# Illumina/manta

Hardware: AMD Instinct MI355X
Metric: candidate SV loci assembled+aligned per second (whole node) (higher is better)
Workload: dtype int32; 1 GPU; BASELINE config[1]: synthetic small-indel loci, 80 reads/locus x150bp, k=31..76 step 5, assemble + 10-mer trim + GlobalLargeIndelAligner(2,-8,-24,-1,-1;-100) on 1800 bp windows; loci_per_gpu=10000, reads_per_locus=80, block_loci=10000, workers_per_gpu=1, parallelism=loci sharded over 1 rank(s); per rank a cost-ordered block queue, queue=rank, dist_world=1, mix=False

## Files before the change

manta_amd/csrc/align_pair.hpp:

```cpp
#pragma once
#include "align_kernels.hpp"

namespace manta_dev {

static const int PAIR_BAD8 = -32768;

WV_HD bool pairEligible(const int E, const int match, const int mismatch, const int open, const int extend, const int offEdge,
                        const int largeIndel, const int allowEdgeIns)
{
  if (E > 6 || allowEdgeIns) return false;
  const long q      = 64L * E;
  const long perCol = -long((mismatch < offEdge) ? ((mismatch < 0) ? mismatch : 0) : ((offEdge < 0) ? offEdge : 0));
  const long gaps   = -long((open < 0) ? open : 0) - long((extend < 0) ? extend : 0) - long((largeIndel < 0) ? largeIndel : 0);
  const long up     = q * long((match > 0) ? match : 0);
  if (open > 0 || extend > 0 || largeIndel > 0 || match < 0 || match > 64 || mismatch < -512 || offEdge < -512 || open < -2048 || largeIndel < -2048 || extend < -512)
    return false;
  const long liftJD = (largeIndel - open > 0) ? long(largeIndel - open) : 0L;
  return q * perCol + gaps + up + liftJD + 64 < 4096;
}

template <int E>
struct PairAligner {
  static const int   NS = 5;
  const AlignParams& P;

  WV_DEV PairAligner(const AlignParams& p) : P(p) {}

  WV_DEV static uint32_t pk(const int lo, const int hi) { return (uint32_t(lo) & 0xffffu) | (uint32_t(hi) << 16); }
  WV_DEV static uint32_t pk2(const int v) { return pk(v, v); }
  WV_DEV static int      half(const uint32_t v, const int h) { return h ? (int(v) >> 16) : int(int16_t(v & 0xffffu)); }

  WV_DEV void sweep(const AlignTaskDev& TA, const AlignTaskDev& TB, uint32_t* ptr32, StartCand& outA, StartCand& outB)
  {
    const int      lane = wv::lane();
    const unsigned QA = TA.query_len, QB = TB.query_len, GA = TA.ref1_len, GB = TB.ref1_len;
    const unsigned G  = (GA > GB) ? GA : GB;
    const int      open = P.open, extend = P.extend, L = P.extra, offEdge = P.off_edge;
    const uint32_t cM0 = pk2(7), cD1 = pk2(6), cI2 = pk2(5), cJ3 = pk2(4), cJI4 = pk2(3);
    const uint32_t cOpen0   = pk2(open * 8 + 7);
    const uint32_t cL0      = pk2(L * 8 + 7);
    const uint32_t cLmOpen2 = pk2((L - open) * 8 + 5);
    const uint32_t cL4      = pk2(L * 8 + 3);
    const uint32_t cBad1 = pk2(PAIR_BAD8 + 6), cBad3 = pk2(PAIR_BAD8 + 4);
    const uint32_t cExt     = pk2(extend * 8);
    const uint32_t cMatch   = pk2(P.match * 8);
    const uint32_t cMisDiff = pk2((P.mismatch - P.match) * 8);
    const uint32_t clrIdx = 0xfff8fff8u, idxBits = 0x00070007u, bad = pk2(PAIR_BAD8);

    const unsigned Qs[2] = {QA, QB}, Gs[2] = {GA, GB};
    unsigned       lQ[2], eQ[2];
    for (int h = 0; h < 2; ++h) {
      lQ[h] = (Qs[h] - 1) / E;
      eQ[h] = (Qs[h] - 1) % E;
    }
    int      rowKey[2] = {int(0x80000000u), int(0x80000000u)};
    uint32_t lastRow[E];
    for (int e = 0; e < E; ++e) lastRow[e] = bad;
    const uint32_t fcMask = (lane == 0) ? 0xffffffffu : 0u;

    uint32_t st[NS][E], lcur[NS], lprev[NS], qc[E];
    for (int e = 0; e < E; ++e) {
      const unsigned q0 = unsigned(lane) * E + e;
      const unsigned a = (q0 < QA) ? TA.query[q0] : 0u, b = (q0 < QB) ? TB.query[q0] : 0u;
      qc[e]            = a | (b << 16);
      const int row0   = int((q0 + 1) * unsigned(offEdge)) * 8;
      for (int s = 0; s < NS; ++s) st[s][e] = bad;
      st[ST_MATCH][e] = pk2(row0 < PAIR_BAD8 ? PAIR_BAD8 : row0);
    }
    for (int s = 0; s < NS; ++s) lcur[s] = lprev[s] = bad;
    lcur[ST_MATCH] = lprev[ST_MATCH] = 0;

    unsigned curA = 0, curB = 0, nextA = 0, nextB = 0;
    {
      const unsigned i0 = unsigned(lane);
      nextA             = (i0 < GA) ? TA.ref1[i0] : 0u;
      nextB             = (i0 < GB) ? TB.ref1[i0] : 0u;
    }
    uint32_t rc = 0;

    const unsigned nSteps = G + 63;
    for (unsigned t = 1; t <= nSteps; ++t) {
      if (((t - 1) & 63) == 0) {
        curA              = nextA;
        curB              = nextB;
        const unsigned i0 = t - 1 + 64 + unsigned(lane);
        nextA             = (i0 < GA) ? TA.ref1[i0] : 0u;
        nextB             = (i0 < GB) ? TB.ref1[i0] : 0u;
      }
      const unsigned c0 = wv::readlane(curA, int((t - 1) & 63)) | (wv::readlane(curB, int((t - 1) & 63)) << 16);
      rc                = wv::shr1(rc, c0);
      uint32_t incoming[NS];
      for (int s = 0; s < NS; ++s) incoming[s] = wv::shr1(st[s][E - 1], (s == ST_MATCH) ? 0u : bad);
      const int g = int(t) - lane;
      for (int s = 0; s < NS; ++s) {
        lprev[s] = lcur[s];
        lcur[s]  = incoming[s];
      }
      const bool active = (g >= 1) && (unsigned(g) <= G);
      if (!active) continue;

      uint32_t diag[NS], left[NS];
      for (int s = 0; s < NS; ++s) {
        diag[s] = lprev[s];
        left[s] = lcur[s];
      }
      uint32_t cells[E];
      for (int e = 0; e < E; ++e) {
        uint32_t up[NS];
        for (int s = 0; s < NS; ++s) up[s] = st[s][e];
        const uint32_t fc = (e == 0) ? fcMask : 0u;
        const uint32_t differ = wv::pk_min_u16(qc[e] ^ rc, 0x00010001u);
        const uint32_t sub8   = wv::pk_mad_u16(differ, cMisDiff, cMatch);
        uint32_t       nv[NS], code;
        {
          uint32_t m = wv::pk_max_i16(wv::pk_max_i16(wv::pk_add_sat_i16(diag[ST_MATCH], cM0), wv::pk_add_sat_i16(diag[ST_DELETE], cD1)), wv::pk_add_sat_i16(diag[ST_INSERT], cI2));
          m          = wv::pk_max_i16(wv::pk_max_i16(m, wv::pk_add_sat_i16(diag[ST_JUMP], cJ3)), wv::pk_add_sat_i16(diag[ST_JUMPINS], cJI4));
          nv[ST_MATCH] = wv::pk_add_sat_i16(m & clrIdx, sub8);
          code         = m & idxBits;
        }
        {
          uint32_t m = wv::pk_max_i16(wv::pk_max_i16(wv::pk_add_sat_i16(up[ST_MATCH], cOpen0), wv::pk_add_sat_i16(up[ST_DELETE], cD1)), wv::pk_add_sat_i16(up[ST_INSERT], cI2));
          m          = wv::pk_max_i16(wv::pk_max_i16(m, cBad3), wv::pk_add_sat_i16(up[ST_JUMPINS], cJI4));
          uint32_t b = wv::pk_add_sat_i16(m & clrIdx, cExt);
          b = (b & ~fc) | (bad & fc);
          nv[ST_DELETE] = b;
          code |= (m & idxBits) << 3;
        }
        {
          uint32_t m = wv::pk_max_i16(wv::pk_max_i16(wv::pk_add_sat_i16(left[ST_MATCH], cOpen0), cBad1), wv::pk_add_sat_i16(left[ST_INSERT], cI2));
          uint32_t b = wv::pk_add_sat_i16(m & clrIdx, cExt);
          b = (b & ~fc) | (bad & fc);
          nv[ST_INSERT] = b;
          code |= (m & idxBits) << 6;
        }
        {
          uint32_t m = wv::pk_max_i16(wv::pk_max_i16(wv::pk_add_sat_i16(up[ST_MATCH], cL0), cBad1), wv::pk_add_sat_i16(up[ST_INSERT], cLmOpen2));
          m          = wv::pk_max_i16(wv::pk_max_i16(m, wv::pk_add_sat_i16(up[ST_JUMP], cJ3)), wv::pk_add_sat_i16(up[ST_JUMPINS], cL4));
          uint32_t b = m & clrIdx;
          b = (b & ~fc) | (bad & fc);
          nv[ST_JUMP] = b;
          code |= (m & idxBits) << 9;
        }
        {
          uint32_t m = wv::pk_max_i16(wv::pk_max_i16(wv::pk_add_sat_i16(left[ST_MATCH], cL0), cBad1), wv::pk_add_sat_i16(left[ST_JUMPINS], cJI4));
          uint32_t b = m & clrIdx;
          b = (b & ~fc) | (bad & fc);
          nv[ST_JUMPINS] = b;
          code |= (m & idxBits) << 12;
        }
        for (int s = 0; s < NS; ++s) {
          diag[s]  = up[s];
          left[s]  = nv[s];
          st[s][e] = nv[s];
        }
        cells[e] = code;
      }
#ifndef MANTA_PAIR_EXPERIMENT_NO_STORE
      for (int e = 0; e < E; ++e) ptr32[(uint64_t(t) * E + e) * 64 + unsigned(lane)] = cells[e];
#else
      if (t == 0xffffffffu) for (int e = 0; e < E; ++e) ptr32[e] = cells[e];
#endif

      {
        const uint32_t cap = ((unsigned(g) == GA) ? 0x0000ffffu : 0u) | ((unsigned(g) == GB) ? 0xffff0000u : 0u);
        for (int e = 0; e < E; ++e) lastRow[e] = (lastRow[e] & ~cap) | (st[ST_MATCH][e] & cap);
        for (int h = 0; h < 2; ++h) {
          uint32_t vM = st[ST_MATCH][0];
          for (int e = 1; e < E; ++e) vM = (unsigned(e) == eQ[h]) ? st[ST_MATCH][e] : vM;
          const int  key = int((uint32_t(half(vM, h)) << 16) | (0xffffu - unsigned(g)));
          const bool on  = unsigned(lane) == lQ[h] && unsigned(g) <= Gs[h];
          rowKey[h]      = imax(rowKey[h], on ? key : int(0x80000000u));
        }
      }
    }
    for (int h = 0; h < 2; ++h) {
      bool     haveOff = false;
      int      offVal  = 0;
      unsigned offQ    = 0;
      for (int e = 0; e < E; ++e) {
        const unsigned q = unsigned(lane) * E + e + 1;
        if (q < Qs[h]) {
          const int v = (half(lastRow[e], h) >> 3) + int((Qs[h] - q) * unsigned(offEdge));
          if (!haveOff || v > offVal) {
            haveOff = true;
            offVal  = v;
            offQ    = q;
          }
        }
      }
      if (lane == 0) {
        const int v0 = int(Qs[h] * unsigned(offEdge));
        if (!haveOff || v0 >= offVal) {
          haveOff = true;
          offVal  = v0;
          offQ    = 0;
        }
      }
      waveArgmaxFirst(haveOff, offVal, offQ);
      const int key = wv::readlane(rowKey[h], int(lQ[h]));
      StartCand best;
      best.val   = (key >> 16) >> 3;
      best.ref   = 0xffffu - (unsigned(key) & 0xffffu);
      best.query = Qs[h];
      best.state = ST_MATCH;
      best.init  = true;
      candUpdate(best, offVal, Gs[h], offQ, ST_MATCH);
      if (h == 0)
        outA = best;
      else
        outB = best;
    }
  }

  WV_DEV void run(const AlignTaskDev& TA, const AlignTaskDev& TB, AlignResultDev& resA, AlignResultDev& resB, const bool haveB, uint8_t* slab)
  {
    StartCand sa, sb;
    sweep(TA, TB, reinterpret_cast<uint32_t*>(slab), sa, sb);
    wv::sync();
    for (int h = 0; h < (haveB ? 2 : 1); ++h) {
      const AlignTaskDev& T = h ? TB : TA;
      Aligner<1, E, true> al(P);
      al.query      = T.query;
      al.ref1       = T.ref1;
      al.ref2       = nullptr;
      al.Q          = T.query_len;
      al.R1         = T.ref1_len;
      al.R2         = 0;
      al.G          = T.ref1_len;
      al.ptr        = reinterpret_cast<uint16_t*>(slab) + h;
      al.nStrips    = 1;
      al.stripCells = 0;
      AlignResultDev r;
      al.tracebackSingle(h ? sb : sa, T, r);
      if (wv::lane() == 0) (h ? resB : resA) = r;
      wv::sync();
    }
  }
};

template <int E>
WV_KERNEL void align_pair_kernel(const AlignParams P)
{
  uint8_t*       slab   = P.ptr_ws + uint64_t(wv::block()) * P.ptr_ws_stride;
  const unsigned nTasks = P.n_tasks_dev ? *P.n_tasks_dev : P.n_tasks;
  const unsigned nPairs = (nTasks + 1) / 2;
  while (true) {
    unsigned slot = 0;
    if (wv::lane() == 0) slot = wv::atomic_add(P.counter, 1u);
    slot = wv::first(slot);
    if (slot >= nPairs) break;
    const unsigned ia = 2 * slot, ib = (2 * slot + 1 < nTasks) ? 2 * slot + 1 : 2 * slot;
    const unsigned ta = P.task_ids ? P.task_ids[ia] : ia, tb = P.task_ids ? P.task_ids[ib] : ib;
    PairAligner<E> al(P);
    al.run(P.tasks[ta], P.tasks[tb], P.results[ta], P.results[tb], ib != ia, slab);
    wv::sync();
  }
}

struct PairMultiParams {
  AlignParams     A;
  const uint32_t* bucket_ids;
  const uint32_t* counts;
  uint32_t        n_slots;
  uint32_t        n_order;
  uint8_t         order[8];
  uint8_t         e_of[8];
  uint32_t        prio_work[3];
};

template <int E>
WV_DEV void runPairWidth(const AlignParams& A, const unsigned ta, const unsigned tb, const bool haveB, uint8_t* slab)
{
  PairAligner<E>(A).run(A.tasks[ta], A.tasks[tb], A.results[ta], A.results[tb], haveB, slab);
}

#if !MANTA_TU_DEFINES(MANTA_TU_ALIGN_PAIR)
WV_KERNEL_OCC(4) void align_pair_multi_kernel(const PairMultiParams M);
#else
WV_KERNEL_OCC(4) void align_pair_multi_kernel(const PairMultiParams M)
{
  uint8_t* slab = M.A.ptr_ws + uint64_t(wv::block()) * M.A.ptr_ws_stride;
  unsigned n0 = 0, n1 = 0, n2 = 0, n3 = 0, n4 = 0, n5 = 0;
  if (M.n_order > 0) n0 = M.counts[M.order[0]];
  if (M.n_order > 1) n1 = M.counts[M.order[1]];
  if (M.n_order > 2) n2 = M.counts[M.order[2]];
  if (M.n_order > 3) n3 = M.counts[M.order[3]];
  if (M.n_order > 4) n4 = M.counts[M.order[4]];
  if (M.n_order > 5) n5 = M.counts[M.order[5]];
  const unsigned f1 = (n0 + 1) / 2, f2 = f1 + (n1 + 1) / 2, f3 = f2 + (n2 + 1) / 2, f4 = f3 + (n3 + 1) / 2, f5 = f4 + (n4 + 1) / 2,
                 f6 = f5 + (n5 + 1) / 2;
  while (true) {
    unsigned slot = 0;
    if (wv::lane() == 0) slot = wv::atomic_add(M.A.counter, 1u);
    slot = wv::first(slot);
    if (slot >= f6) break;
    unsigned j = 0, base = 0, n = n0;
    if (slot >= f1) { j = 1; base = f1; n = n1; }
    if (slot >= f2) { j = 2; base = f2; n = n2; }
    if (slot >= f3) { j = 3; base = f3; n = n3; }
    if (slot >= f4) { j = 4; base = f4; n = n4; }
    if (slot >= f5) { j = 5; base = f5; n = n5; }
    const unsigned  p   = slot - base;
    const uint32_t* ids = M.bucket_ids + uint64_t(M.order[j]) * M.n_slots;
    const unsigned  ia = 2 * p, ib = (2 * p + 1 < n) ? 2 * p + 1 : 2 * p;
    const unsigned  ta = ids[ia], tb = ids[ib];
    {
      const unsigned ga = M.A.tasks[ta].ref1_len, gb = M.A.tasks[tb].ref1_len;
      const unsigned work = unsigned(M.e_of[j]) * (((ga > gb) ? ga : gb) + 64u);
      wv::setprio((M.prio_work[2] && work >= M.prio_work[2]) ? 3u : (M.prio_work[1] && work >= M.prio_work[1]) ? 2u : (M.prio_work[0] && work >= M.prio_work[0]) ? 1u : 0u);
    }
    switch (M.e_of[j]) {
    case 1: runPairWidth<1>(M.A, ta, tb, ib != ia, slab); break;
    case 2: runPairWidth<2>(M.A, ta, tb, ib != ia, slab); break;
    case 3: runPairWidth<3>(M.A, ta, tb, ib != ia, slab); break;
    case 4: runPairWidth<4>(M.A, ta, tb, ib != ia, slab); break;
    case 5: runPairWidth<5>(M.A, ta, tb, ib != ia, slab); break;
    default: runPairWidth<6>(M.A, ta, tb, ib != ia, slab); break;
    }
    wv::sync();
  }
}
#endif

#if MANTA_TU != MANTA_TU_ALL
#if MANTA_TU == MANTA_TU_ALIGN_PAIR
#define MANTA_X
#else
#define MANTA_X extern
#endif
MANTA_X template __global__ void align_pair_kernel<1>(const AlignParams);
MANTA_X template __global__ void align_pair_kernel<2>(const AlignParams);
MANTA_X template __global__ void align_pair_kernel<3>(const AlignParams);
MANTA_X template __global__ void align_pair_kernel<4>(const AlignParams);
MANTA_X template __global__ void align_pair_kernel<5>(const AlignParams);
MANTA_X template __global__ void align_pair_kernel<6>(const AlignParams);
#undef MANTA_X
#endif

}
```

manta_amd/csrc/api.cpp:

```cpp
#include "api_internal.hpp"

extern "C" {

uint32_t manta_abi_version(void) { return MANTA_ABI_VERSION; }
uint64_t manta_batch_stats_size(void) { return sizeof(manta_batch_stats_t); }

int manta_ctx_create(int device_id, manta_ctx_t** out)
{
  if (!out) {
    g_createError = "manta_ctx_create: null output pointer";
    return MANTA_E_INVALID_ARG;
  }
  *out = nullptr;
  try {
    rt::init(device_id);
    if (!stringHashMatchesLibstdcxx()) {
      g_createError = "this libstdc++'s std::hash<std::string> is not the Murmur variant the exact repeat search restates";
      return MANTA_E_UNSUPPORTED;
    }
    manta_ctx_t* ctx = new manta_ctx();
    ctx->deviceName  = rt::deviceName();
    ctx->cuCount     = rt::cuCount();
    ctx->deviceId    = rt::currentDevice();
    *out             = ctx;
// ... 439 lines not shown
  if (n_loci == 0 || !refs || !ref_off || !cuts) return fail(ctx, MANTA_E_INVALID_ARG, "manta_smallsv_upload_piles: null argument or empty batch");
  int rc = checkPiles(ctx, piles, "manta_smallsv_upload_piles");
  if (rc != MANTA_OK) return rc;
  try {
    rt::setDevice(ctx->deviceId);
    rt::ScopedStream onStream(b->main);
    b->uploaded = false;
    b->refsOnCopy = false;
    rc          = b->asmStage.plan(b->opt, n_loci, nullptr, piles->locus_read_begin, piles->read_len);
    if (rc != MANTA_OK) return rc;
    b->nLoci    = n_loci;
    b->refBytes = ref_off[n_loci];
    b->maxRef   = 0;
    for (uint32_t l = 0; l < n_loci; ++l) {
      if (ref_off[l + 1] < ref_off[l]) return fail(ctx, MANTA_E_INVALID_ARG, "manta_smallsv_upload_piles: ref_off not monotone");
      b->maxRef = std::max<uint64_t>(b->maxRef, ref_off[l + 1] - ref_off[l]);
      if (cuts[l].leading_cut < 0 || cuts[l].trailing_cut < 0 || cuts[l].max_leading_cut < 0 || cuts[l].max_trailing_cut < 0)
        return fail(ctx, MANTA_E_INVALID_ARG, "manta_smallsv_upload_piles: negative reference cut");
    }
    uint8_t*  dRefs   = b->dRefs.as<uint8_t>(b->refBytes + 16);
    uint64_t* dRefOff = b->dRefOff.as<uint64_t>(n_loci + 1);
    auto*     dCuts   = b->dCuts.as<SmallSvCuts>(n_loci);
    b->refsOnCopy     = b->streamUploads && !std::getenv("MANTA_AMD_NO_STREAM_UPLOAD");
    if (b->refsOnCopy) {
      b->asmStage.uploadPilesStreamed(*piles, b->copy);
      rt::ScopedStream onCopy(b->copy);
      rt::h2d(dRefs, refs, b->refBytes);
      rt::h2d(dRefOff, ref_off, sizeof(uint64_t) * (n_loci + 1));
      rt::h2d(dCuts, cuts, sizeof(SmallSvCuts) * n_loci);
      b->refsReady.record();
    } else {
      b->asmStage.uploadPiles(*piles);
      rt::h2d(dRefs, refs, b->refBytes);
      rt::h2d(dRefOff, ref_off, sizeof(uint64_t) * (n_loci + 1));
      rt::h2d(dCuts, cuts, sizeof(SmallSvCuts) * n_loci);
      rt::sync();
    }
    b->uploaded = true;
    return MANTA_OK;
  } catch (const std::exception& e) {
    return fail(ctx, MANTA_E_HIP, e.what());
  }
}

}

int smallsvRunImpl(manta_smallsv_t* b, StageGates* gates)
{
  if (!b) return MANTA_E_INVALID_ARG;
  manta_ctx_t* ctx = b->ctx;
  if (!b->uploaded) return fail(ctx, MANTA_E_INVALID_ARG, "manta_smallsv_run: nothing uploaded");
  try {
    rt::setDevice(ctx->deviceId);
    rt::ScopedStream onStream(b->main);
    const uint32_t nLoci   = b->nLoci;
    const uint32_t maxAsm  = b->opt.max_assembly_count;
    const uint64_t nSlots  = uint64_t(nLoci) * maxAsm;
    AsmStage&      as(b->asmStage);
    AlignTaskDev*    dTasks   = b->dTasks.as<AlignTaskDev>(nSlots);
    SmallSvTaskInfo* dInfo    = b->dInfo.as<SmallSvTaskInfo>(nSlots);
    AlignResultDev*  dResults = b->dResults.as<AlignResultDev>(nSlots);
    uint32_t*        dBuckets = b->dBucketIds.as<uint32_t>(nSlots * kNumESet);
    uint32_t*        dSmall   = b->dSmall.as<uint32_t>(64);
    const uint32_t   tableCap = nextPow2(2ull * as.maxContigLen);
    const int        schedWaves = std::getenv("MANTA_AMD_SCHED_WAVES_PER_CU") ? std::max(1, std::atoi(std::getenv("MANTA_AMD_SCHED_WAVES_PER_CU"))) : 12;
    const uint32_t   schedChunk = std::getenv("MANTA_AMD_SCHED_CHUNK") ? uint32_t(std::max(1, std::atoi(std::getenv("MANTA_AMD_SCHED_CHUNK")))) : 2u;
    const int        schedGrid = rt::roundGrid(int(std::min<uint64_t>((nLoci + schedChunk - 1) / schedChunk, uint64_t(std::max(1, ctx->cuCount * schedWaves)))));
    uint32_t*        dTable   = b->dTable.as<uint32_t>(uint64_t(tableCap) * schedGrid);
    rt::dzero(dSmall, sizeof(uint32_t) * 64);
    rt::dzero(dResults, sizeof(AlignResultDev) * nSlots);

    const bool dbg = std::getenv("MANTA_AMD_DEBUG") != nullptr;
    auto       stage = [&](const char* what) {
      if (!dbg) return;
      rt::sync();
      std::fprintf(stderr, "manta_amd: smallsv_run %s\n", what);
      std::fflush(stderr);
    };
    stage("start");
    uint64_t asmCnt[4];
    {
      GateLock only(gates, &StageGates::asmMu);
      std::unique_lock<std::mutex> streamedOnly(streamedAsmMu(ctx), std::defer_lock);
      if (as.chunks.active()) streamedOnly.lock();
      as.stageQueued = false;
      as.earlyStaged = false;
      b->evStart.record();
      as.launch();
      b->evAsm.record();
      rt::d2h(asmCnt, as.dCnt, sizeof(asmCnt));
      if (asmCnt[3]) {
        as.rerunCapacityFailures(asmCnt[3]);
        rt::d2h(asmCnt, as.dCnt, sizeof(asmCnt));
      }
    }
    stage("assembled");
    const bool noEarlyStage = std::getenv("MANTA_AMD_NO_EARLY_STAGE") != nullptr;
    const bool        earlyStage   = b->stageBehindRun && b->whileAligning && !noEarlyStage;
    if (earlyStage) as.stageEarly(b->copy, asmCnt, b->evEarlyStaged);
    const uint64_t cigarCap = 8ull * std::min<uint64_t>(asmCnt[1], as.devSeqCap) + 64;
    if (cigarCap + 16 > 0xffffffffull)
      return fail(ctx, MANTA_E_UNSUPPORTED, "manta_smallsv_run: alignment scratch of this block exceeds 2^32 words; use smaller blocks "
                                         "(manta_smallsv_batch splits a batch into blocks, manta_batch_plan_t::block_loci)");
    uint32_t* dCigar = b->dCigar.as<uint32_t>(cigarCap + 16);
    GateLock alignOnly(gates, &StageGates::alignMu);
    if (b->refsOnCopy) rt::curStreamWaits(b->refsReady);

    ScheduleParams S;
    S.loci               = as.dLoci;
    S.contigs            = as.dCont;
    S.seq_arena          = as.dSeq;
    S.n_loci             = nLoci;
    S.max_assembly_count = maxAsm;
    S.refs               = static_cast<const uint8_t*>(b->dRefs.p);
    S.ref_off            = static_cast<const uint64_t*>(b->dRefOff.p);
    S.cuts               = static_cast<const SmallSvCuts*>(b->dCuts.p);
    S.tasks              = dTasks;
    S.info               = dInfo;
    S.bucket_ids         = dBuckets;
    S.bucket_count       = dSmall;
    S.bucket_maxref      = dSmall + 16;
    S.cigar_used         = reinterpret_cast<unsigned long long*>(dSmall + 34);
    S.cigar_cap          = cigarCap;
    S.counter            = dSmall + 32;
    S.table_ws           = dTable;
    S.table_cap          = tableCap;
    S.n_e                = kNumESet;
    S.chunk              = schedChunk;
    for (int i = 0; i < kNumESet; ++i) S.e_set[i] = uint32_t(kESet[i]);
    rt::launch(smallsv_schedule_kernel, schedGrid, SCHED_LDS_BYTES, S);
    uint32_t  pairMask       = 0;
    uint32_t* dBucketsSorted = nullptr;
    for (int k = 0; k < kNumESet; ++k)
      if (alignUsesPairs(MANTA_ALIGNER_LARGE_INDEL, k, b->scores.match, b->scores.mismatch, b->scores.open, b->scores.extend, b->scores.off_edge,
                         b->largeIndel, b->scores.is_allow_edge_insertion ? 1 : 0, b->maxRef))
        pairMask |= 1u << k;
    if (pairMask) {
      dBucketsSorted = b->dBucketIds2.as<uint32_t>(nSlots * kNumESet);
      BucketSortParams BS;
      BS.tasks        = dTasks;
      BS.loci         = as.dLoci;
      BS.info         = dInfo;
      BS.ids_out      = dBucketsSorted;
      BS.n_loci       = nLoci;
      BS.max_assembly_count = maxAsm;
      BS.total        = uint32_t(nSlots);
      BS.mask         = pairMask;
      rt::launchWG(bucket_sort_kernel, kNumESet, int(BS_WAVES), BS_LDS_BYTES, BS);
    }
    b->evSched.record();
    stage("scheduled");

    uint32_t hSmall[40];
    const int    maxWaves = std::max(1, ctx->cuCount * alignWavesPerCu());
    const size_t wsBudget = workspaceBudget(size_t(48) << 30);
    bool         fromHistory = b->bucketHistory && b->stageBehindRun && !std::getenv("MANTA_AMD_SYNC_BUCKETS");
    struct Launch {
      int      k, grid;
      uint64_t stride, slabOff;
      bool     pair;
    };
    std::vector<Launch> launches;
    uint64_t            slabBytes = 0;
    auto pairOf = [&](int k) {
      return alignUsesPairs(MANTA_ALIGNER_LARGE_INDEL, k, b->scores.match, b->scores.mismatch, b->scores.open, b->scores.extend, b->scores.off_edge,
                            b->largeIndel, b->scores.is_allow_edge_insertion ? 1 : 0, b->maxRef);
    };
    const bool batchCall = b->stageBehindRun && !std::getenv("MANTA_AMD_SYNC_BUCKETS");
    bool       haveCounts = false;
    if (batchCall && !fromHistory) {
      rt::d2h(hSmall, dSmall, sizeof(hSmall));
      std::memcpy(b->lastSmall, hSmall, sizeof(b->lastSmall));
      haveCounts  = true;
      fromHistory = true;
    }
    if (fromHistory) {
      for (int k = kNumESet - 1; k >= 0; --k) {
        const bool     pair   = pairOf(k);
        const uint64_t tasks  = b->lastSmall[k] ? uint64_t(b->lastSmall[k]) + b->lastSmall[k] / 4 + 64 : 4;
        const uint64_t hint   = pair ? (tasks + 1) / 2 : tasks;
        const uint64_t qBound = (kESet[k] == 32) ? std::max<uint64_t>(as.maxContigLen, 64ull * 32) : 64ull * uint64_t(kESet[k]);
        const uint64_t refLen = alignSlabRefLen(MANTA_ALIGNER_LARGE_INDEL, kESet[k], qBound, b->maxRef);
        const uint64_t stride = ((pair ? 2 : 1) * alignPtrSlabBytes(MANTA_ALIGNER_LARGE_INDEL, kESet[k], refLen) + 255) & ~uint64_t(255);
        const int      grid   = rt::roundGrid(int(std::min<uint64_t>(hint, uint64_t(maxWaves))));
        launches.push_back(Launch{k, grid, stride, slabBytes, pair});
        slabBytes += stride * uint64_t(grid);
      }
      if (slabBytes > wsBudget / 3) {
        fromHistory = false;
        launches.clear();
        slabBytes = 0;
      }
    }
    if (!fromHistory) {
      if (!haveCounts) rt::d2h(hSmall, dSmall, sizeof(hSmall));
      for (int k = kNumESet - 1; k >= 0; --k) {
        const uint32_t cnt = hSmall[k];
        if (cnt == 0) continue;
        const bool     pair   = pairOf(k);
        const uint64_t stride = ((pair ? 2 : 1) * alignPtrSlabBytes(MANTA_ALIGNER_LARGE_INDEL, kESet[k], hSmall[16 + k]) + 255) & ~uint64_t(255);
        int            grid   = int(std::min<size_t>(pair ? (cnt + 1) / 2 : cnt, size_t(maxWaves)));
        grid                  = int(std::max<size_t>(1, std::min<size_t>(size_t(grid), (wsBudget / 3) / stride)));
        grid                  = rt::roundGrid(grid);
        launches.push_back(Launch{k, grid, stride, slabBytes, pair});
        slabBytes += stride * uint64_t(grid);
      }
    }
    b->stats.n_align_launches = 0;
    b->stats.n_alignments     = 0;
    b->stats.ptr_matrix_bytes = 0;
    {
      static const bool   noMerge = std::getenv("MANTA_AMD_NO_ALIGN_MERGE") != nullptr;
      std::vector<Launch> merged;
      if (!noMerge) {
        std::vector<Launch> rest;
        for (const Launch& l : launches) (l.pair ? merged : rest).push_back(l);
        if (merged.size() < 2 || merged.size() > 6) {
          merged.clear();
        } else {
          launches.swap(rest);
          slabBytes = 0;
          for (Launch& l : launches) {
            l.slabOff = slabBytes;
            slabBytes += l.stride * uint64_t(l.grid);
          }
        }
      }
      uint64_t mergedStride = 0, mergedWaves = 0, mergedOff = slabBytes;
      const uint32_t* counts = fromHistory ? b->lastSmall : hSmall;
      if (!merged.empty()) {
        std::stable_sort(merged.begin(), merged.end(), [&](const Launch& x, const Launch& y) { return counts[x.k] < counts[y.k]; });
        for (const Launch& l : merged) {
          mergedStride = std::max(mergedStride, l.stride);
          mergedWaves += uint64_t(l.grid);
        }
        mergedWaves = std::min<uint64_t>(std::min<uint64_t>(mergedWaves, uint64_t(maxWaves)), (wsBudget / 3) / mergedStride);
        mergedWaves = std::max<uint64_t>(WV_WAVES_PER_WG, (mergedWaves / WV_WAVES_PER_WG) * WV_WAVES_PER_WG);
        slabBytes += mergedStride * mergedWaves;
      }
      uint8_t* dWsAll = b->dPtrWs.as<uint8_t>(slabBytes + 256);
      for (int i = 0; i < 3; ++i) rt::streamWaits(b->side[i], b->evSched);
      auto baseParams = [&]() {
        AlignParams P;
        P.tasks          = dTasks;
        P.results        = dResults;
        P.cigar          = dCigar;
        P.task_ids       = nullptr;
        P.n_tasks        = 0;
        P.n_tasks_dev    = nullptr;
        P.counter        = nullptr;
        P.ptr_ws         = nullptr;
        P.ptr_ws_stride  = 0;
        P.match          = b->scores.match;
        P.mismatch       = b->scores.mismatch;
        P.open           = b->scores.open;
        P.extend         = b->scores.extend;
        P.off_edge       = b->scores.off_edge;
        P.allow_edge_ins = b->scores.is_allow_edge_insertion ? 1 : 0;
        P.extra          = b->largeIndel;
        return P;
      };
      for (size_t i = 0; i < launches.size(); ++i) {
        const Launch& l(launches[i]);
        AlignParams   P  = baseParams();
        P.task_ids       = (l.pair ? dBucketsSorted : dBuckets) + uint64_t(l.k) * nSlots;
        P.n_tasks        = fromHistory ? uint32_t(nSlots) : hSmall[l.k];
        P.n_tasks_dev    = fromHistory ? dSmall + l.k : nullptr;
        P.counter        = dSmall + 40 + l.k;
        P.ptr_ws         = dWsAll + l.slabOff;
        P.ptr_ws_stride  = l.stride;
        {
          rt::ScopedStream onSide(b->side[i % 3]);
          launchAlignKind(MANTA_ALIGNER_LARGE_INDEL, l.k, l.grid, P, l.pair);
        }
        if (!fromHistory) {
          b->stats.n_align_launches++;
          b->stats.n_alignments += hSmall[l.k];
        }
      }
      if (!merged.empty()) {
        PairMultiParams M;
        M.A               = baseParams();
        M.A.counter       = dSmall + 40 + merged[0].k;
        M.A.ptr_ws        = dWsAll + mergedOff;
        M.A.ptr_ws_stride = mergedStride;
        M.bucket_ids      = dBucketsSorted;
        M.counts          = dSmall;
        M.n_slots         = uint32_t(nSlots);
        M.n_order         = uint32_t(merged.size());
        M.prio_work[0] = 2560u;
        M.prio_work[1] = 0u;
        M.prio_work[2] = 4096u;
        if (const char* e = std::getenv("MANTA_AMD_ALIGN_PRIO")) {
          unsigned v[3] = {0, 0, 0};
          std::sscanf(e, "%u,%u,%u", &v[0], &v[1], &v[2]);
          for (int i = 0; i < 3; ++i) M.prio_work[i] = v[i];
        }
        for (size_t i = 0; i < 8; ++i) {
          M.order[i] = uint8_t(i < merged.size() ? merged[i].k : 0);
          M.e_of[i]  = uint8_t(i < merged.size() ? kESet[merged[i].k] : 0);
        }
        if (std::getenv("MANTA_AMD_DEBUG"))
          std::fprintf(stderr, "manta_amd: align_pair_multi_kernel: %llu waves over %zu packed buckets, slab stride %llu\n",
                       (unsigned long long)mergedWaves, merged.size(), (unsigned long long)mergedStride);
        rt::launch(align_pair_multi_kernel, int(mergedWaves), 0, M);
        if (!fromHistory) {
          b->stats.n_align_launches++;
// ... 561 lines not shown
```

manta_amd/csrc/api_internal.hpp:

```cpp
#pragma once
#include "../../include/manta_amd.h"

#include <algorithm>
#include <atomic>
#include <functional>
#include <condition_variable>
#include <chrono>
#include <cstdio>
#include <cstdlib>
#include <cstring>
#include <memory>
#include <mutex>
#include <optional>
#include <string>
#include <thread>
#include <vector>

#include "align_kernels.hpp"
#include "align_jump_pair.hpp"
#include "assemble_kernels.hpp"
#include "asm_lds.hpp"
#include "small_asm.hpp"
#include "pipeline_kernels.hpp"
#include "split_kernels.hpp"
// ... 59 lines not shown
  }
};

inline double nowMs()
{
  return std::chrono::duration<double, std::milli>(std::chrono::steady_clock::now().time_since_epoch()).count();
}

inline std::atomic<int> g_liveWorkspaces{0};

}
#include "upload_stream.hpp"
using namespace manta_host;

struct manta_smallsv;
struct manta_spanning;

struct manta_ctx {
  std::mutex  errMu;
  std::string lastError;
  std::string deviceName;
  int         cuCount = 0;
  DevBuf dSeq, dTasks, dResults, dCigar, dTaskIds, dCounter, dPtrWs, dTaskFlags;
  DevBuf dSplitTasks, dSplitResults, dSplitTables;
  DevBuf dRc[16];
  DevBuf dQc[6];
  rt::Stream stream;
  int        deviceId = 0;
  std::vector<manta_smallsv*>  smallPool;
  std::vector<manta_spanning*> spanPool;
  ~manta_ctx();
  std::vector<uint32_t> growthSize, growthBuckets;
  std::once_flag         growthOnce;
};

namespace manta_host {

inline int fail(manta_ctx_t* ctx, int code, const std::string& msg)
{
  if (ctx) {
    std::lock_guard<std::mutex> g(ctx->errMu);
    ctx->lastError = msg;
  }
  return code;
}

inline bool perItemCode(int rc)
{
  return rc == MANTA_E_UNSUPPORTED || rc == MANTA_E_DEVICE_FAULT || rc == MANTA_E_EMPTY_SEQ;
}

inline std::string lastErrorOf(manta_ctx_t* ctx)
{
  std::lock_guard<std::mutex> g(ctx->errMu);
  return ctx->lastError;
}

const int kESet[]  = {1, 2, 3, 4, 5, 6, 8, 10, 12, 16, 24, 32};
const int kNumESet = sizeof(kESet) / sizeof(kESet[0]);

inline int pickE(uint32_t qlen)
{
  const uint32_t need = (qlen + 63) / 64;
  for (int i = 0; i < kNumESet; ++i)
    if (uint32_t(kESet[i]) >= need) return i;
  return kNumESet - 1;
}

template <int KIND, int E>
void launchAlign(int grid, const AlignParams& P)
{
  rt::launch(align_kernel<KIND, E>, grid, 0, P);
}

template <int KIND>
void launchAlignE(int eIdx, int grid, const AlignParams& P)
{
  switch (kESet[eIdx]) {
  case 1: launchAlign<KIND, 1>(grid, P); break;
  case 2: launchAlign<KIND, 2>(grid, P); break;
  case 3: launchAlign<KIND, 3>(grid, P); break;
  case 4: launchAlign<KIND, 4>(grid, P); break;
  case 5: launchAlign<KIND, 5>(grid, P); break;
  case 6: launchAlign<KIND, 6>(grid, P); break;
  case 8: launchAlign<KIND, 8>(grid, P); break;
  case 10: launchAlign<KIND, 10>(grid, P); break;
  case 12: launchAlign<KIND, 12>(grid, P); break;
  case 16: launchAlign<KIND, 16>(grid, P); break;
  case 24: launchAlign<KIND, 24>(grid, P); break;
  case 32: launchAlign<KIND, 32>(grid, P); break;
  default: throw rt::Error("internal: unsupported E");
  }
}

inline bool alignUsesPairs(int kind, int eIdx, int match, int mismatch, int open, int extend, int offEdge, int extra, int allowEdgeIns, uint64_t maxRef)
{
  static const bool off = std::getenv("MANTA_AMD_NO_ALIGN_PAIRS") != nullptr;
  static const bool offJump = std::getenv("MANTA_AMD_NO_JUMP_PAIRS") != nullptr;
  if (off || maxRef > 0xfffeu) return false;
  if (kind == MANTA_ALIGNER_LARGE_INDEL) return pairEligible(kESet[eIdx], match, mismatch, open, extend, offEdge, extra, allowEdgeIns);
  if (kind == MANTA_ALIGNER_JUMP) return !offJump && !allowEdgeIns && jumpPairEligible(kESet[eIdx], match, mismatch, open, extend, offEdge, extra);
  return false;
}

inline void launchJumpPair(int eIdx, int grid, const AlignParams& P)
{
  if (std::getenv("MANTA_AMD_DEBUG")) std::fprintf(stderr, "manta_amd: align_jump_pair_kernel<%d>: %d waves (two alignments each)\n", kESet[eIdx], grid);
  switch (kESet[eIdx]) {
  case 1: rt::launch(align_jump_pair_kernel<1>, grid, 0, P); break;
  case 2: rt::launch(align_jump_pair_kernel<2>, grid, 0, P); break;
  case 3: rt::launch(align_jump_pair_kernel<3>, grid, 0, P); break;
  case 4: rt::launch(align_jump_pair_kernel<4>, grid, 0, P); break;
  case 5: rt::launch(align_jump_pair_kernel<5>, grid, 0, P); break;
  case 6: rt::launch(align_jump_pair_kernel<6>, grid, 0, P); break;
  case 8: rt::launch(align_jump_pair_kernel<8>, grid, 0, P); break;
  default: throw rt::Error("internal: no packed jump aligner for this E");
  }
}

inline void launchAlignPair(int eIdx, int grid, const AlignParams& P)
{
  if (std::getenv("MANTA_AMD_DEBUG")) std::fprintf(stderr, "manta_amd: align_pair_kernel<%d>: %d waves (two alignments each)\n", kESet[eIdx], grid);
  switch (kESet[eIdx]) {
  case 1: rt::launch(align_pair_kernel<1>, grid, 0, P); break;
  case 2: rt::launch(align_pair_kernel<2>, grid, 0, P); break;
  case 3: rt::launch(align_pair_kernel<3>, grid, 0, P); break;
  case 4: rt::launch(align_pair_kernel<4>, grid, 0, P); break;
  case 5: rt::launch(align_pair_kernel<5>, grid, 0, P); break;
  case 6: rt::launch(align_pair_kernel<6>, grid, 0, P); break;
  default: throw rt::Error("internal: no packed aligner for this E");
  }
}

inline void launchAlignKind(int kind, int eIdx, int grid, const AlignParams& P, bool pair = false)
{
  if (kind == MANTA_ALIGNER_GLOBAL)
    launchAlignE<0>(eIdx, grid, P);
  else if (kind == MANTA_ALIGNER_LARGE_INDEL) {
    if (pair)
      launchAlignPair(eIdx, grid, P);
    else
      launchAlignE<1>(eIdx, grid, P);
  } else if (kind == MANTA_ALIGNER_JUMP_INTRON)
    launchAlignE<3>(eIdx, grid, P);
  else if (pair)
    launchJumpPair(eIdx, grid, P);
  else
    launchAlignE<2>(eIdx, grid, P);
}

inline int alignWavesPerCu()
{
  return std::getenv("MANTA_AMD_ALIGN_WAVES_PER_CU") ? std::atoi(std::getenv("MANTA_AMD_ALIGN_WAVES_PER_CU")) : 16;
}

inline void recordGrowthSchedule(std::vector<uint32_t>& sizes, std::vector<uint32_t>& buckets, const uint32_t upTo)
{
  std::unordered_map<int, int> m;
  size_t                       last = m.bucket_count();
  for (uint32_t i = 0; i < upTo; ++i) {
    m[int(i)] = 0;
    if (m.bucket_count() != last) {
      sizes.push_back(i);
      buckets.push_back(uint32_t(m.bucket_count()));
      last = m.bucket_count();
    }
  }
}

inline bool stringHashMatchesLibstdcxx()
{
  auto mix = [](uint64_t v) { return v ^ (v >> 47); };
  const char* probes[] = {"A", "ACGTACG", "ACGTACGT", "ACGTTGCAAGCTTGACCATGGTACCAGTCAGT", "TTTTTTTTTTTTTTTTTTTTTTTTTTTTTTTTTTTTTTTTTGACGATCGATCGTAGCTAGCTAGCTAGCTAGCTAGTCG"};
  for (const char* p : probes) {
    const std::string s(p);
    const uint64_t    mul  = (uint64_t(0xc6a4a793UL) << 32) + uint64_t(0x5bd1e995UL);
    uint64_t          hash = uint64_t(0xc70f6907UL) ^ (uint64_t(s.size()) * mul);
    const size_t      al   = s.size() & ~size_t(7);
    for (size_t i = 0; i < al; i += 8) {
      uint64_t d = 0;
      for (int b = 0; b < 8; ++b) d |= uint64_t(uint8_t(s[i + b])) << (8 * b);
      d = mix(d * mul) * mul;
      hash ^= d;
      hash *= mul;
    }
    if (s.size() & 7) {
      uint64_t d = 0;
      for (size_t b = 0; b < (s.size() & 7); ++b) d |= uint64_t(uint8_t(s[al + b])) << (8 * b);
      hash ^= d;
      hash *= mul;
    }
    hash = mix(hash) * mul;
    hash = mix(hash);
    if (hash != uint64_t(std::hash<std::string>()(s))) return false;
  }
  return true;
}

static const int kMaxDevices = 64;
inline std::atomic<int> g_livePerDevice[kMaxDevices];
inline size_t workspaceBudget(const size_t capBytes)
{
  static std::mutex                            mu;
  static size_t                                cachedFree[kMaxDevices] = {0};
  static std::chrono::steady_clock::time_point stamp[kMaxDevices];
  const int                                    dev = std::min(kMaxDevices - 1, std::max(0, rt::currentDevice()));
  size_t                                       freeNow;
  {
    std::lock_guard<std::mutex> g(mu);
    const auto                  now = std::chrono::steady_clock::now();
    if (cachedFree[dev] == 0 || now - stamp[dev] > std::chrono::milliseconds(250)) {
      cachedFree[dev] = rt::freeBytes();
      stamp[dev]      = now;
    }
    freeNow = cachedFree[dev];
  }
  const int live = std::max(1, g_livePerDevice[dev].load());
  return std::min<size_t>(freeNow / 2 / size_t(live), capBytes);
}

#define MANTA_SCAN_OFFSETS_BODY                                                      \
  uint64_t w = 0, mw = 0, hi = 0;                                                    \
  uint32_t m = 0;                                                                    \
  for (uint32_t i = 0; i < n; ++i) {                                                 \
    const uint64_t len = o[i + 1] - o[i];                                            \
    w += (len + 15) >> 4;                                                            \
    mw += (len + 31) >> 5;                                                           \
    hi |= len >> 32;                                                                 \
    const uint32_t l32 = uint32_t(len);                                              \
    m                  = m > l32 ? m : l32;                                          \
  }                                                                                  \
  wOut       = w;                                                                    \
  mwOut      = mw;                                                                   \
  longestOut = hi ? ~uint64_t(0) : uint64_t(m);
inline void scanOffsetsBase(const uint64_t* o, const uint32_t n, uint64_t& wOut, uint64_t& mwOut, uint64_t& longestOut) { MANTA_SCAN_OFFSETS_BODY }
#if defined(__x86_64__) && !defined(MANTA_NO_AVX2_SCAN)
__attribute__((target("avx2"))) inline void scanOffsetsAvx2(const uint64_t* o, const uint32_t n, uint64_t& wOut, uint64_t& mwOut, uint64_t& longestOut) { MANTA_SCAN_OFFSETS_BODY }
inline bool hostHasAvx2()
{
  static const bool has = __builtin_cpu_supports("avx2") != 0;
  return has;
}
#else
inline void scanOffsetsAvx2(const uint64_t* o, const uint32_t n, uint64_t& wOut, uint64_t& mwOut, uint64_t& longestOut) { MANTA_SCAN_OFFSETS_BODY }
inline bool hostHasAvx2() { return false; }
#endif
#undef MANTA_SCAN_OFFSETS_BODY

inline uint32_t nextPow2(uint64_t v)
{
  uint64_t p = 1;
  while (p < v) p <<= 1;
  return uint32_t(p);
}

inline int asmStatusToAbi(int st)
{
  switch (st) {
  case ASM_OK: return MANTA_OK;
  case ASM_E_ALPHABET:
  case ASM_E_WORD_TOO_LONG:
  case ASM_E_TOO_MANY_READS: return MANTA_E_UNSUPPORTED;
  default: return MANTA_E_DEVICE_FAULT;
  }
}


struct AsmStage {
  manta_ctx_t* ctx;
  explicit AsmStage(manta_ctx_t* c) : ctx(c)
  {
    g_liveWorkspaces++;
    g_livePerDevice[std::min(kMaxDevices - 1, std::max(0, c->deviceId))]++;
  }
  ~AsmStage()
  {
    g_liveWorkspaces--;
    g_livePerDevice[std::min(kMaxDevices - 1, std::max(0, ctx->deviceId))]--;
  }
  AsmStage(const AsmStage&) = delete;
  AsmStage& operator=(const AsmStage&) = delete;
  PinnedBuf     pLoci, pCont, pSeq, pBits, pCnt;
  AsmLocusOut*  hLoci = nullptr;
  AsmContigOut* hCont = nullptr;
  uint8_t*      hSeq  = nullptr;
  uint64_t*     hBits = nullptr;
  uint64_t*     hCnt  = nullptr;
  uint64_t      seqUsedDev = 0, bitsUsedDev = 0, nContigsOut = 0, pseudoBytesOut = 0, pseudoCountOut = 0;
  bool          staged = false;
  uint32_t      ldsFallbacks = 0;

  manta_asm_options_t opt{};
  uint32_t            nLoci = 0, nReadsTotal = 0, maxContigLen = 0, wMax = 0, capWords = 0, capReads = 0, capNodes = 0, capSlots = 0;
  uint64_t            nBases = 0, stride = 0, devSeqCap = 0, devBitsCap = 0;
  int                 grid = 1;
  DevBuf              bBases, bReadOff, bLocusBegin, bLoci, bContigs, bSeqArena, bBitsArena, bCounters, bWs, bGrowth, bWl, bOrder;
  std::vector<uint32_t> locusMinWl, locusMaxWl;
  std::vector<uint32_t> order;
  uint32_t              maxWordLen = 0;
  uint32_t              capWords2 = 0, capNodes2 = 0, capSlots2 = 0;
  uint64_t              stride2 = 0;
  DevBuf                bWs2, bFailIds;
  uint32_t              nRerun = 0;
  AsmParams             lastParams{};
  bool                  smallMode = false;
  uint32_t              smallMinSeedReads = 0, smallMaxIterations = 0;
// ... 1517 lines not shown
```

Baseline: 1.205 million loci/s.

## Pre-tag pair aligner scores with source state, trim sweep steps, retune occupancy

```diff
diff --git a/manta_amd/csrc/align_pair.hpp b/manta_amd/csrc/align_pair.hpp
--- a/manta_amd/csrc/align_pair.hpp
+++ b/manta_amd/csrc/align_pair.hpp
@@ -36,25 +36,28 @@
     const unsigned QA = TA.query_len, QB = TB.query_len, GA = TA.ref1_len, GB = TB.ref1_len;
     const unsigned G  = (GA > GB) ? GA : GB;
     const int      open = P.open, extend = P.extend, L = P.extra, offEdge = P.off_edge;
-    const uint32_t cM0 = pk2(7), cD1 = pk2(6), cI2 = pk2(5), cJ3 = pk2(4), cJI4 = pk2(3);
-    const uint32_t cOpen0   = pk2(open * 8 + 7);
-    const uint32_t cL0      = pk2(L * 8 + 7);
-    const uint32_t cLmOpen2 = pk2((L - open) * 8 + 5);
-    const uint32_t cL4      = pk2(L * 8 + 3);
-    const uint32_t cBad1 = pk2(PAIR_BAD8 + 6), cBad3 = pk2(PAIR_BAD8 + 4);
-    const uint32_t cExt     = pk2(extend * 8);
-    const uint32_t cMatch   = pk2(P.match * 8);
+    const uint32_t cOpen    = pk2(open * 8);
+    const uint32_t cL       = pk2(L * 8);
+    const uint32_t cLmOpen  = pk2((L - open) * 8);
+    const uint32_t cExtD    = pk2(extend * 8 + (7 - ST_DELETE));
+    const uint32_t cExtI    = pk2(extend * 8 + (7 - ST_INSERT));
+    const uint32_t cMatch   = pk2(P.match * 8 + (7 - ST_MATCH));
     const uint32_t cMisDiff = pk2((P.mismatch - P.match) * 8);
+    const uint32_t tagJ = pk2(7 - ST_JUMP), tagJI = pk2(7 - ST_JUMPINS), tagM = pk2(7 - ST_MATCH);
     const uint32_t clrIdx = 0xfff8fff8u, idxBits = 0x00070007u, bad = pk2(PAIR_BAD8);
 
     const unsigned Qs[2] = {QA, QB}, Gs[2] = {GA, GB};
-    unsigned       lQ[2], eQ[2];
+    unsigned       lQ[2], eQ[2], tKeyEnd[2];
     for (int h = 0; h < 2; ++h) {
-      lQ[h] = (Qs[h] - 1) / E;
-      eQ[h] = (Qs[h] - 1) % E;
-    }
-    int      rowKey[2] = {int(0x80000000u), int(0x80000000u)};
-    uint32_t lastRow[E];
+      lQ[h]      = (Qs[h] - 1) / E;
+      eQ[h]      = (Qs[h] - 1) % E;
+      tKeyEnd[h] = Gs[h] + lQ[h];
+    }
+    uint32_t selQ[E];
+    for (int e = 0; e < E; ++e) selQ[e] = ((unsigned(e) == eQ[0]) ? 0x0000ffffu : 0u) | ((unsigned(e) == eQ[1]) ? 0xffff0000u : 0u);
+    const unsigned tCapLo = (GA < GB) ? GA : GB, tCapHi = G + 63;
+    int            rowKey[2] = {int(0x80000000u), int(0x80000000u)};
+    uint32_t       lastRow[E];
     for (int e = 0; e < E; ++e) lastRow[e] = bad;
     const uint32_t fcMask = (lane == 0) ? 0xffffffffu : 0u;
 
@@ -65,10 +68,10 @@
       qc[e]            = a | (b << 16);
       const int row0   = int((q0 + 1) * unsigned(offEdge)) * 8;
       for (int s = 0; s < NS; ++s) st[s][e] = bad;
-      st[ST_MATCH][e] = pk2(row0 < PAIR_BAD8 ? PAIR_BAD8 : row0);
+      st[ST_MATCH][e] = pk2(row0 < PAIR_BAD8 ? PAIR_BAD8 : row0 + (7 - ST_MATCH));
     }
     for (int s = 0; s < NS; ++s) lcur[s] = lprev[s] = bad;
-    lcur[ST_MATCH] = lprev[ST_MATCH] = 0;
+    lcur[ST_MATCH] = lprev[ST_MATCH] = tagM;
 
     unsigned curA = 0, curB = 0, nextA = 0, nextB = 0;
     {
@@ -78,7 +81,7 @@
     }
     uint32_t rc = 0;
 
-    const unsigned nSteps = G + 63;
+    const unsigned nSteps = G + ((lQ[0] > lQ[1]) ? lQ[0] : lQ[1]);
     for (unsigned t = 1; t <= nSteps; ++t) {
       if (((t - 1) & 63) == 0) {
         curA              = nextA;
@@ -90,7 +93,7 @@
       const unsigned c0 = wv::readlane(curA, int((t - 1) & 63)) | (wv::readlane(curB, int((t - 1) & 63)) << 16);
       rc                = wv::shr1(rc, c0);
       uint32_t incoming[NS];
-      for (int s = 0; s < NS; ++s) incoming[s] = wv::shr1(st[s][E - 1], (s == ST_MATCH) ? 0u : bad);
+      for (int s = 0; s < NS; ++s) incoming[s] = wv::shr1(st[s][E - 1], (s == ST_MATCH) ? tagM : bad);
       const int g = int(t) - lane;
       for (int s = 0; s < NS; ++s) {
         lprev[s] = lcur[s];
@@ -111,43 +114,45 @@
         const uint32_t fc = (e == 0) ? fcMask : 0u;
         const uint32_t differ = wv::pk_min_u16(qc[e] ^ rc, 0x00010001u);
         const uint32_t sub8   = wv::pk_mad_u16(differ, cMisDiff, cMatch);
-        uint32_t       nv[NS], code;
-        {
-          uint32_t m = wv::pk_max_i16(wv::pk_max_i16(wv::pk_add_sat_i16(diag[ST_MATCH], cM0), wv::pk_add_sat_i16(diag[ST_DELETE], cD1)), wv::pk_add_sat_i16(diag[ST_INSERT], cI2));
-          m          = wv::pk_max_i16(wv::pk_max_i16(m, wv::pk_add_sat_i16(diag[ST_JUMP], cJ3)), wv::pk_add_sat_i16(diag[ST_JUMPINS], cJI4));
+        uint32_t       nv[NS], tag[NS];
+        {
+          uint32_t m = wv::pk_max_i16(wv::pk_max_i16(diag[ST_MATCH], diag[ST_DELETE]), diag[ST_INSERT]);
+          m          = wv::pk_max_i16(wv::pk_max_i16(m, diag[ST_JUMP]), diag[ST_JUMPINS]);
           nv[ST_MATCH] = wv::pk_add_sat_i16(m & clrIdx, sub8);
-          code         = m & idxBits;
-        }
-        {
-          uint32_t m = wv::pk_max_i16(wv::pk_max_i16(wv::pk_add_sat_i16(up[ST_MATCH], cOpen0), wv::pk_add_sat_i16(up[ST_DELETE], cD1)), wv::pk_add_sat_i16(up[ST_INSERT], cI2));
-          m          = wv::pk_max_i16(wv::pk_max_i16(m, cBad3), wv::pk_add_sat_i16(up[ST_JUMPINS], cJI4));
-          uint32_t b = wv::pk_add_sat_i16(m & clrIdx, cExt);
+          tag[ST_MATCH] = m & idxBits;
+        }
+        {
+          uint32_t m = wv::pk_max_i16(wv::pk_max_i16(wv::pk_add_sat_i16(up[ST_MATCH], cOpen), up[ST_DELETE]), up[ST_INSERT]);
+          m          = wv::pk_max_i16(m, up[ST_JUMPINS]);
+          uint32_t b = wv::pk_add_sat_i16(m & clrIdx, cExtD);
           b = (b & ~fc) | (bad & fc);
           nv[ST_DELETE] = b;
-          code |= (m & idxBits) << 3;
-        }
-        {
-          uint32_t m = wv::pk_max_i16(wv::pk_max_i16(wv::pk_add_sat_i16(left[ST_MATCH], cOpen0), cBad1), wv::pk_add_sat_i16(left[ST_INSERT], cI2));
-          uint32_t b = wv::pk_add_sat_i16(m & clrIdx, cExt);
+          tag[ST_DELETE] = m & idxBits;
+        }
+        {
+          uint32_t m = wv::pk_max_i16(wv::pk_add_sat_i16(left[ST_MATCH], cOpen), left[ST_INSERT]);
+          uint32_t b = wv::pk_add_sat_i16(m & clrIdx, cExtI);
           b = (b & ~fc) | (bad & fc);
           nv[ST_INSERT] = b;
-          code |= (m & idxBits) << 6;
-        }
-        {
-          uint32_t m = wv::pk_max_i16(wv::pk_max_i16(wv::pk_add_sat_i16(up[ST_MATCH], cL0), cBad1), wv::pk_add_sat_i16(up[ST_INSERT], cLmOpen2));
-          m          = wv::pk_max_i16(wv::pk_max_i16(m, wv::pk_add_sat_i16(up[ST_JUMP], cJ3)), wv::pk_add_sat_i16(up[ST_JUMPINS], cL4));
-          uint32_t b = m & clrIdx;
+          tag[ST_INSERT] = m & idxBits;
+        }
+        {
+          uint32_t m = wv::pk_max_i16(wv::pk_add_sat_i16(up[ST_MATCH], cL), wv::pk_add_sat_i16(up[ST_INSERT], cLmOpen));
+          m          = wv::pk_max_i16(wv::pk_max_i16(m, up[ST_JUMP]), wv::pk_add_sat_i16(up[ST_JUMPINS], cL));
+          uint32_t b = (m & clrIdx) | tagJ;
           b = (b & ~fc) | (bad & fc);
           nv[ST_JUMP] = b;
-          code |= (m & idxBits) << 9;
-        }
-        {
-          uint32_t m = wv::pk_max_i16(wv::pk_max_i16(wv::pk_add_sat_i16(left[ST_MATCH], cL0), cBad1), wv::pk_add_sat_i16(left[ST_JUMPINS], cJI4));
-          uint32_t b = m & clrIdx;
+          tag[ST_JUMP] = m & idxBits;
+        }
+        {
+          uint32_t m = wv::pk_max_i16(wv::pk_add_sat_i16(left[ST_MATCH], cL), left[ST_JUMPINS]);
+          uint32_t b = (m & clrIdx) | tagJI;
           b = (b & ~fc) | (bad & fc);
           nv[ST_JUMPINS] = b;
-          code |= (m & idxBits) << 12;
-        }
+          tag[ST_JUMPINS] = m & idxBits;
+        }
+        uint32_t code = tag[NS - 1];
+        for (int s = NS - 2; s >= 0; --s) code = (code << 3) | tag[s];
         for (int s = 0; s < NS; ++s) {
           diag[s]  = up[s];
           left[s]  = nv[s];
@@ -161,16 +166,16 @@
       if (t == 0xffffffffu) for (int e = 0; e < E; ++e) ptr32[e] = cells[e];
 #endif
 
-      {
+      if (t >= tCapLo && t <= tCapHi) {
         const uint32_t cap = ((unsigned(g) == GA) ? 0x0000ffffu : 0u) | ((unsigned(g) == GB) ? 0xffff0000u : 0u);
         for (int e = 0; e < E; ++e) lastRow[e] = (lastRow[e] & ~cap) | (st[ST_MATCH][e] & cap);
-        for (int h = 0; h < 2; ++h) {
-          uint32_t vM = st[ST_MATCH][0];
-          for (int e = 1; e < E; ++e) vM = (unsigned(e) == eQ[h]) ? st[ST_MATCH][e] : vM;
-          const int  key = int((uint32_t(half(vM, h)) << 16) | (0xffffu - unsigned(g)));
-          const bool on  = unsigned(lane) == lQ[h] && unsigned(g) <= Gs[h];
-          rowKey[h]      = imax(rowKey[h], on ? key : int(0x80000000u));
-        }
+      }
+      {
+        uint32_t vM = st[ST_MATCH][0];
+        for (int e = 1; e < E; ++e) vM = (st[ST_MATCH][e] & selQ[e]) | (vM & ~selQ[e]);
+        const uint32_t rowInv = 0xffffu - unsigned(g);
+        if (t <= tKeyEnd[0]) rowKey[0] = imax(rowKey[0], int((vM << 16) | rowInv));
+        if (t <= tKeyEnd[1]) rowKey[1] = imax(rowKey[1], int((vM & 0xffff0000u) | rowInv));
       }
     }
     for (int h = 0; h < 2; ++h) {
@@ -274,10 +279,13 @@
   PairAligner<E>(A).run(A.tasks[ta], A.tasks[tb], A.results[ta], A.results[tb], haveB, slab);
 }
 
+#ifndef MANTA_PAIR_MULTI_OCC
+#define MANTA_PAIR_MULTI_OCC 3
+#endif
 #if !MANTA_TU_DEFINES(MANTA_TU_ALIGN_PAIR)
-WV_KERNEL_OCC(4) void align_pair_multi_kernel(const PairMultiParams M);
+WV_KERNEL_OCC(MANTA_PAIR_MULTI_OCC) void align_pair_multi_kernel(const PairMultiParams M);
 #else
-WV_KERNEL_OCC(4) void align_pair_multi_kernel(const PairMultiParams M)
+WV_KERNEL_OCC(MANTA_PAIR_MULTI_OCC) void align_pair_multi_kernel(const PairMultiParams M)
 {
   uint8_t* slab = M.A.ptr_ws + uint64_t(wv::block()) * M.A.ptr_ws_stride;
   unsigned n0 = 0, n1 = 0, n2 = 0, n3 = 0, n4 = 0, n5 = 0;
diff --git a/manta_amd/csrc/api.cpp b/manta_amd/csrc/api.cpp
--- a/manta_amd/csrc/api.cpp
+++ b/manta_amd/csrc/api.cpp
@@ -615,7 +615,7 @@
     stage("scheduled");
 
     uint32_t hSmall[40];
-    const int    maxWaves = std::max(1, ctx->cuCount * alignWavesPerCu());
+    const int    maxWaves = std::max(1, ctx->cuCount * smallsvAlignWavesPerCu());
     const size_t wsBudget = workspaceBudget(size_t(48) << 30);
     bool         fromHistory = b->bucketHistory && b->stageBehindRun && !std::getenv("MANTA_AMD_SYNC_BUCKETS");
     struct Launch {
diff --git a/manta_amd/csrc/api_internal.hpp b/manta_amd/csrc/api_internal.hpp
--- a/manta_amd/csrc/api_internal.hpp
+++ b/manta_amd/csrc/api_internal.hpp
@@ -235,6 +235,11 @@
 inline int alignWavesPerCu()
 {
   return std::getenv("MANTA_AMD_ALIGN_WAVES_PER_CU") ? std::atoi(std::getenv("MANTA_AMD_ALIGN_WAVES_PER_CU")) : 16;
+}
+
+inline int smallsvAlignWavesPerCu()
+{
+  return std::getenv("MANTA_AMD_ALIGN_WAVES_PER_CU") ? std::atoi(std::getenv("MANTA_AMD_ALIGN_WAVES_PER_CU")) : 4 * MANTA_PAIR_MULTI_OCC;
 }
 
 inline void recordGrowthSchedule(std::vector<uint32_t>& sizes, std::vector<uint32_t>& buckets, const uint32_t upTo)
```

Result: faster. 1.287 million loci/s, median of 6 (+6.8%).
